# yanx27/PointASNL

Measured on AMD Instinct MI355X. Metric: point-clouds/sec fwd (Bx1024 pts, ModelNet40 cls), higher is better.
Workload: dtype f32; 1 GPU; configs[1]: ModelNet40 pointasnl_cls, 1024 pts, batch=64/GPU, seeded random weights; global_batch=64, parallelism=batch-shard x1, RCCL all-gather of logits, pipeline=prefetch, hip_graph=True, prefix_forked_at=start, prefix_levels=2, settle_replays=40, hip_hw_queues=4

## Files before the change

### include/pasnl.h

```cpp
#ifndef PASNL_H_
#define PASNL_H_

#include <stddef.h>
#include <stdint.h>

#ifdef __cplusplus
extern "C" {
#endif

#define PASNL_VERSION 100

enum {
  PASNL_OK = 0,
  PASNL_EINVAL = -1,
  PASNL_ENULL = -2,
  PASNL_EWORKSPACE = -3,
  PASNL_ELAUNCH = -4,
  PASNL_EUNSUPPORTED = -5
};

typedef void* pasnl_stream_t;

int pasnl_version(void);
const char* pasnl_strerror(int code);
// ... 102 lines not shown

int pasnl_sa_cell_packed(int b, int n, int c, int npoint, int nsample, int c1, int c2, const float* xyz, const float* feature,
                         const int* idx, const float* new_xyz, const float* w0, const float* b0, const float* w1, const float* b1,
                         const float* ww, const float* bw, const float* w0_features_packed, const float* w1_packed, float* out,
                         float* skip_max, float* new_xyz_out, float* new_feature_out, pasnl_stream_t stream);

int pasnl_max_pool_rows(int b, int n, int c, const float* x, float* out, pasnl_stream_t stream);

int pasnl_max_pool_rows_strided(int b, int n, int c, const float* x, float* out, long out_stride, pasnl_stream_t stream);

size_t pasnl_mlp3_packed_weights_bytes(int k, int n);
int pasnl_mlp3_pack_weights(int k, int n, const float* w, float* packed, pasnl_stream_t stream);
size_t pasnl_mlp3_max_pool_workspace_bytes(int b, int n, int c3);
int pasnl_mlp3_max_pool(int b, int n, int k0, int c1, int c2, int c3, const float* x, const float* w0, const float* b0,
                        const float* w1, const float* b1, const float* w2, const float* b2, float* out, long out_stride,
                        void* workspace, size_t workspace_bytes, pasnl_stream_t stream);

int pasnl_cls_tail_group_all(int b, int n, int w, int cb, int c, const float* after, const float* skip_max, const float* att,
                             const float* ws_packed, const float* bs, const float* wb_packed, const float* bb,
                             const float* wagg_packed, const float* bagg, const float* new_xyz, int c1, int c2, int c3,
                             const float* w0, const float* b0, const float* w1, const float* b1, const float* w2, const float* b2,
                             float* out, float* pooled, long pooled_stride, void* workspace, size_t workspace_bytes,
                             pasnl_stream_t stream);

size_t pasnl_bf16x3_weights_bytes(int kdim, int n);
int pasnl_bf16x3_split_weights(int kdim, int n, const float* w, void* wsplit, pasnl_stream_t stream);
int pasnl_dense_bf16x3(int rows, int kdim, int n, int lda, const float* x, const void* wsplit, const float* bias, int relu,
                       float* out, pasnl_stream_t stream);


size_t pasnl_dense_rows_workspace_bytes(int rows, int kdim, int n);
int pasnl_dense_rows(int rows, int kdim, int n, const float* x, const float* w, const float* bias, int relu, float* out,
                     void* workspace, size_t workspace_bytes, pasnl_stream_t stream);

size_t pasnl_dense_splitk_workspace_bytes(int rows, int kdim, int n);
int pasnl_dense_splitk(int rows, int kdim, int n, int lda, const float* x, const float* w, const float* bias, int relu,
                       float* out, void* workspace, size_t workspace_bytes, pasnl_stream_t stream);

int pasnl_narrow_project2(long rows0, int kdim0, int n0, const float* x0, const float* w0, const float* bias0, float* out0,
                          long rows1, int kdim1, int n1, const float* x1, const float* w1, const float* bias1, float* out1,
                          pasnl_stream_t stream);

size_t pasnl_grad_workspace_bytes(int b, int targets, long contributions);
int pasnl_gather_point_grad_det(int b, int n, int m, const float* out_g, const int* idx, float* inp_g, void* workspace,
                                size_t workspace_bytes, pasnl_stream_t stream);
int pasnl_group_point_grad_det(int b, int n, int c, int m, int nsample, const float* grad_out, const int* idx,
// ... 252 lines not shown
```

### pointasnl_amd/_hip.py

```python
import ctypes
import os

import torch

_HERE = os.path.dirname(os.path.abspath(__file__))
LIB_PATH = os.path.join(_HERE, "csrc", "libpasnl_hip.so")

SYMBOLS = [
    "pasnl_version", "pasnl_strerror", "pasnl_device_count",
    "pasnl_farthest_point_sample", "pasnl_farthest_point_sample_gather", "pasnl_gather_point", "pasnl_gather_point_grad", "pasnl_prob_sample",
    "pasnl_query_ball_point", "pasnl_sa_group", "pasnl_group_point", "pasnl_group_point_grad", "pasnl_select_top_k", "pasnl_knn_batch", "pasnl_knn_workspace_bytes", "pasnl_knn_batch_ws", "pasnl_knn_batch_ws_bg", "pasnl_knn_tree_workspace_bytes", "pasnl_knn_batch_tree", "pasnl_knn_batch_ref_workspace_bytes", "pasnl_knn_batch_ref", "pasnl_knn_distance_pick",
    "pasnl_three_nn", "pasnl_three_interpolate", "pasnl_three_interpolate_grad", "pasnl_three_weights", "pasnl_fp_interpolate_cat",
    "pasnl_nl_attention", "pasnl_nl_attention_workspace_bytes", "pasnl_nl_attention_ws", "pasnl_as_attention", "pasnl_as_reweight", "pasnl_sa_local_cell", "pasnl_sa_cell", "pasnl_sa_cell_centre0", "pasnl_sa_cell_packed", "pasnl_sa_project", "pasnl_sa_cell_pre", "pasnl_sa_cell_pre_centre0", "pasnl_sa_tail", "pasnl_sa_tail_cat", "pasnl_sa_tail_res", "pasnl_sa_tail_packed_weights_bytes", "pasnl_sa_tail_pack_weights", "pasnl_sa_tail_packed", "pasnl_decode_cell", "pasnl_decode_cell_tiled", "pasnl_decode_cell_tiled_v4", "pasnl_max_pool_rows", "pasnl_max_pool_rows_strided", "pasnl_mlp3_max_pool_workspace_bytes", "pasnl_mlp3_max_pool", "pasnl_mlp3_packed_weights_bytes", "pasnl_mlp3_pack_weights", "pasnl_dense_rows_workspace_bytes", "pasnl_dense_rows", "pasnl_dense_splitk_workspace_bytes", "pasnl_dense_splitk", "pasnl_bf16x3_weights_bytes", "pasnl_bf16x3_split_weights", "pasnl_dense_bf16x3", "pasnl_narrow_project2", "pasnl_take_neighbor0", "pasnl_as_gather", "pasnl_as_attention_qkv", "pasnl_as_attention_proj", "pasnl_as_cell_narrow", "pasnl_as_cell_wide", "pasnl_as_cell_wide_ld", "pasnl_as_reweight_x", "pasnl_grid_subsample_workspace_bytes", "pasnl_grid_subsample", "pasnl_knn_crop_workspace_bytes", "pasnl_knn_crop",
    "pasnl_scan_pick", "pasnl_knn_crop_indirect", "pasnl_crop_order_permute", "pasnl_scan_possibility_update", "pasnl_scan_scratch_init", "pasnl_scan_vote", "pasnl_scan_reproject_workspace_bytes", "pasnl_scan_reproject", "pasnl_scan_labels",
    "pasnl_scan_pick_given", "pasnl_scan_train_labels", "pasnl_scan_augment",
    "pasnl_scene_pick", "pasnl_knn_crop_scene", "pasnl_scene_pick_crop", "pasnl_scene_order_gather", "pasnl_scene_potential_update", "pasnl_scene_vote", "pasnl_scene_labels", "pasnl_confusion_matrix",
    "pasnl_window_noise", "pasnl_window_bounds", "pasnl_window_hist_bytes", "pasnl_window_count", "pasnl_window_fill", "pasnl_window_gather", "pasnl_window_vote", "pasnl_window_pool_labels",
    "pasnl_kwindow_hist_bytes", "pasnl_kwindow_count", "pasnl_kwindow_fill", "pasnl_kwindow_gather",
    "pasnl_modelnet_fps_cap", "pasnl_modelnet_fps", "pasnl_modelnet_normalize", "pasnl_modelnet_batch", "pasnl_modelnet_augment", "pasnl_modelnet_noise", "pasnl_cls_vote", "pasnl_cls_tally",
    "pasnl_cls_tail_group_all",
    "pasnl_block_key_capacity", "pasnl_block_crop_stats", "pasnl_block_grid_count", "pasnl_block_fill", "pasnl_block_gather", "pasnl_block_normalize", "pasnl_block_score_workspace_bytes", "pasnl_block_score", "pasnl_block_train_batch", "pasnl_block_train_score",
    "pasnl_kblock_crop_stats", "pasnl_kblock_grid_count", "pasnl_kblock_fill", "pasnl_kblock_gather", "pasnl_kblock_rotate",
    "pasnl_grad_workspace_bytes", "pasnl_gather_point_grad_det", "pasnl_group_point_grad_det", "pasnl_three_interpolate_grad_det",
]


class PasnlError(RuntimeError):
    pass


class PasnlUnsupported(PasnlError):
    """PASNL_EUNSUPPORTED: a valid request outside what the fused kernel covers (include/pasnl.h documents the limits).
    The cells catch it and take their op-by-op path (still HIP kernels + vendor GEMMs, never a CPU path)."""


_lib = None


def lib():
    global _lib
    if _lib is None:
        if not os.path.exists(LIB_PATH):
            raise PasnlError(
                f"{LIB_PATH} is missing: build it with `python -c 'import __graft_entry__ as g; g.build()'` "
                "(or `make -C pointasnl_amd/csrc`).  pointasnl_amd has no CPU or eager fallback.")
        _lib = ctypes.CDLL(LIB_PATH)
        _lib.pasnl_strerror.restype = ctypes.c_char_p
        _lib.pasnl_grad_workspace_bytes.restype = ctypes.c_size_t
        _lib.pasnl_knn_workspace_bytes.restype = ctypes.c_size_t
        _lib.pasnl_knn_tree_workspace_bytes.restype = ctypes.c_size_t
        _lib.pasnl_knn_batch_ref_workspace_bytes.restype = ctypes.c_size_t
        _lib.pasnl_dense_rows_workspace_bytes.restype = ctypes.c_size_t
        _lib.pasnl_bf16x3_weights_bytes.restype = ctypes.c_size_t
        _lib.pasnl_mlp3_max_pool_workspace_bytes.restype = ctypes.c_size_t
        _lib.pasnl_mlp3_packed_weights_bytes.restype = ctypes.c_size_t
        _lib.pasnl_sa_tail_packed_weights_bytes.restype = ctypes.c_size_t
        _lib.pasnl_dense_splitk_workspace_bytes.restype = ctypes.c_size_t
        _lib.pasnl_grid_subsample_workspace_bytes.restype = ctypes.c_size_t
        _lib.pasnl_knn_crop_workspace_bytes.restype = ctypes.c_size_t
        _lib.pasnl_scan_reproject_workspace_bytes.restype = ctypes.c_size_t
        _lib.pasnl_nl_attention_workspace_bytes.restype = ctypes.c_size_t
        _lib.pasnl_window_hist_bytes.restype = ctypes.c_size_t
        _lib.pasnl_kwindow_hist_bytes.restype = ctypes.c_size_t
        _lib.pasnl_block_score_workspace_bytes.restype = ctypes.c_size_t
        for s in SYMBOLS:
            getattr(_lib, s)
    return _lib


def require_device():
    if not torch.cuda.is_available():
        raise PasnlError("no HIP device visible: pointasnl_amd runs on MI355X (gfx950) only and has no CPU fallback")


def stream_ptr():
    return ctypes.c_void_p(torch.cuda.current_stream().cuda_stream)


def ptr(t, byte_offset=0):
# ... 92 lines not shown
```

### pointasnl_amd/csrc/mlp_pool.hip

```cpp
#include "common.hpp"
#include "sa_tail.hpp"

namespace pasnl {

typedef float mp_f32x16 __attribute__((ext_vector_type(16)));

__device__ __forceinline__ int mp_kappa(int t, int h) { return (t & 3) + 8 * (t >> 2) + 4 * h; }

template <int WOUT, int NB, int RB>
__device__ __forceinline__ void mp_mm(const float* xrow, int rbstride, int NBT, const float* __restrict__ Wp, const int (&loff)[NB],
                                      mp_f32x16 (&acc)[RB][NB]) {
  constexpr int BT = 8;
  float xb[2][RB][BT];
  float4 wa[2][NB][2];
  auto load = [&](int set, int bt) {
    const float* wrow = Wp + (size_t)bt * (16 * WOUT);
#pragma unroll
    for (int i = 0; i < NB; ++i) {
      wa[set][i][0] = *reinterpret_cast<const float4*>(wrow + loff[i]);
      wa[set][i][1] = *reinterpret_cast<const float4*>(wrow + loff[i] + 4);
    }
#pragma unroll
    for (int u = 0; u < BT; ++u)
#pragma unroll
// ... 40 lines not shown
  if (wave >= BLOCKS) return;
  int loff[NB];
  mp_f32x16 acc[RB][NB];
#pragma unroll
  for (int i = 0; i < NB; ++i) {
    loff[i] = (h * WOUT + (wave + NW * i) * 32 + ql) * 8;
#pragma unroll
    for (int rb = 0; rb < RB; ++rb)
#pragma unroll
      for (int r = 0; r < 16; ++r) acc[rb][i][r] = 0.f;
  }
  mp_mm<WOUT, NB, RB>(in + ql * pin + h, 32 * pin, (K + 15) >> 4, W, loff, acc);
#pragma unroll
  for (int i = 0; i < NB; ++i) {
    const int ch = (wave + NW * i) * 32 + ql;
    const float bb = bias[ch];
#pragma unroll
    for (int rb = 0; rb < RB; ++rb)
#pragma unroll
      for (int r = 0; r < 16; ++r) out[(rb * 32 + mp_kappa(r, h)) * pout + ch] = fmaxf(acc[rb][i][r] + bb, 0.f);
  }
}

template <int C1, int C2, int C3, int RB>
__device__ __forceinline__ void mlp3_tile(float* A, int pa, float* Bf, int k0, const float* __restrict__ w0, const float* __restrict__ b0,
                                          const float* __restrict__ w1, const float* __restrict__ b1, const float* __restrict__ w2,
                                          const float* __restrict__ b2, float* __restrict__ po, int wave, int ql, int h) {
  constexpr int NW = 8, PB = C1 + 1;
  mp_layer<C1, RB>(A, pa, k0, w0, b0, Bf, PB, wave, ql, h);
  __syncthreads();
  mp_layer<C2, RB>(Bf, PB, C1, w1, b1, A, pa, wave, ql, h);
  __syncthreads();
  constexpr int NB = C3 / 32 / NW;
  int loff[NB];
  mp_f32x16 acc[RB][NB];
#pragma unroll
  for (int i = 0; i < NB; ++i) {
    loff[i] = (h * C3 + (wave + NW * i) * 32 + ql) * 8;
#pragma unroll
    for (int rb = 0; rb < RB; ++rb)
#pragma unroll
      for (int r = 0; r < 16; ++r) acc[rb][i][r] = 0.f;
  }
  mp_mm<C3, NB, RB>(A + ql * pa + h, 32 * pa, C2 >> 4, w2, loff, acc);
#pragma unroll
  for (int i = 0; i < NB; ++i) {
    float mx = acc[0][i][0];
#pragma unroll
    for (int rb = 0; rb < RB; ++rb)
#pragma unroll
      for (int r = 0; r < 16; ++r) mx = fmaxf(mx, acc[rb][i][r]);
    mx = fmaxf(mx, __shfl_xor(mx, 32));
    const int ch = (wave + NW * i) * 32 + ql;
    if (h == 0) po[ch] = fmaxf(mx + b2[ch], 0.f);
  }
}

template <int C1, int C2, int C3, int RB>
__global__ __launch_bounds__(512) void mlp3_pool_kernel(int n, int k0, const float* __restrict__ x, const float* __restrict__ w0,
                                                        const float* __restrict__ b0, const float* __restrict__ w1,
                                                        const float* __restrict__ b1, const float* __restrict__ w2,
                                                        const float* __restrict__ b2, float* __restrict__ partial) {
  constexpr int NW = 8;
  static_assert(C1 % 32 == 0 && C2 % 256 == 0 && C3 % 256 == 0, "blocks of 32 channels; the two wide layers fill all eight waves");
  extern __shared__ __attribute__((aligned(16))) char smem[];
  const int pa = max((k0 + 15) & ~15, C2) | 1;
  constexpr int TR = 32 * RB;
  float* A = reinterpret_cast<float*>(smem);
  float* Bf = A + TR * pa;
  const int tid = threadIdx.x, lane = tid & 63, wave = tid >> 6, h = lane >> 5, ql = lane & 31;
  const int tile = blockIdx.x, cloud = blockIdx.y;
  {
    const int q4 = k0 >> 2;
    const float4* xc = reinterpret_cast<const float4*>(x + (size_t)cloud * n * k0);
    for (int r = wave; r < TR; r += NW) {
      const int row = min(tile * TR + r, n - 1);
      for (int q = lane; q < q4; q += 64) {
        const float4 v = xc[(size_t)row * q4 + q];
        float* d = A + r * pa + 4 * q;
        d[0] = v.x; d[1] = v.y; d[2] = v.z; d[3] = v.w;
      }
      if (lane < ((k0 + 15) & ~15) - k0) A[r * pa + k0 + lane] = 0.f;
    }
  }
  __syncthreads();
  mlp3_tile<C1, C2, C3, RB>(A, pa, Bf, k0, w0, b0, w1, b1, w2, b2, partial + ((size_t)cloud * gridDim.x + tile) * C3, wave, ql, h);
}

constexpr int TG_C = 128, TG_W = 9, TG_CB = 32, TG_K0 = TG_C + 4, TG_C2 = 256, TG_C3 = 512, TG_TR = 64;
constexpr int TG_PA = (((TG_K0 + 15) & ~15) > TG_C2 ? ((TG_K0 + 15) & ~15) : TG_C2) | 1;
constexpr int TG_TAIL_FLOATS = 2 * (TG_C + 32 + 32) * 33;
constexpr int TG_H1_FLOATS = TG_TR * (TG_C + 1);
constexpr size_t TG_LDS_BYTES = ((size_t)TG_TR * TG_PA + (TG_TAIL_FLOATS > TG_H1_FLOATS ? TG_TAIL_FLOATS : TG_H1_FLOATS)) * sizeof(float);
static_assert(TG_LDS_BYTES <= LDS_MAX_BYTES, "X rows + the tail's tiles fit one workgroup's LDS");
static_assert(TG_W <= 2 * TAIL_KS && TG_CB == 2 * TAIL_KS && TG_C % 64 == 0 && TG_C / 32 * 2 == 8, "one (channel block, row block) per wave");

__global__ __launch_bounds__(512) void tail_group_all_kernel(int n, const float* __restrict__ after, const float* __restrict__ S,
                                                             const float* __restrict__ N, const float* __restrict__ Ws,
                                                             const float* __restrict__ bs, const float* __restrict__ Wb,
                                                             const float* __restrict__ bb, const float* __restrict__ Wagg,
                                                             const float* __restrict__ bagg, const float* __restrict__ xyz3,
                                                             const float* __restrict__ w0, const float* __restrict__ b0,
                                                             const float* __restrict__ w1, const float* __restrict__ b1,
                                                             const float* __restrict__ w2, const float* __restrict__ b2,
                                                             float* __restrict__ out, float* __restrict__ partial) {
  constexpr int C = TG_C, pa = TG_PA, RPW = TG_TR / 8;
  extern __shared__ __attribute__((aligned(16))) char smem[];
  float* A = reinterpret_cast<float*>(smem);
  float* Bf = A + TG_TR * pa;
  const int tid = threadIdx.x, lane = tid & 63, wave = tid >> 6, h = lane >> 5, l32 = lane & 31;
  const int tile = blockIdx.x, cloud = blockIdx.y;
  const long cloud0 = (long)cloud * n;
  const int rb = wave >> 2;
  float* vt = Bf + rb * (C * 33);
  float* st = Bf + 2 * C * 33 + rb * (32 * 33);
  float* nt_ = Bf + 2 * (C + 32) * 33 + rb * (32 * 33);
  {
    float v[3][RPW], cx[RPW];
#pragma unroll
    for (int i = 0; i < RPW; ++i) {
      const long row = cloud0 + min(tile * TG_TR + wave * RPW + i, n - 1);
      v[0][i] = after[row * C + lane];
      v[1][i] = after[row * C + 64 + lane];
      v[2][i] = h ? N[row * TG_CB + l32] : S[row * TG_W + min(l32, TG_W - 1)];
      cx[i] = xyz3[row * 3 + max(min(lane, 3) - 1, 0)];
    }
    __builtin_amdgcn_sched_barrier(0);
    const int rr0 = (wave & 3) * RPW;
// ... 28 lines not shown
      *cell = *cell + v[i];
    }
  }
  __syncthreads();
  {
    f32x16 o;
#pragma unroll
    for (int i = 0; i < 16; ++i) o[i] = bagg[cbase + kappa(i, h)];
    o = tail_product(TailW<true>{Wagg, C, C, h, cbase + l32}, vt, l32, o);
    float* xr = A + (rb * 32 + l32) * pa + 4 + cbase;
#pragma unroll
    for (int i = 0; i < 16; ++i) xr[kappa(i, h)] = fmaxf(o[i], 0.f);
  }
  __syncthreads();
#pragma unroll
  for (int i = 0; i < RPW; ++i) {
    const int r = wave * RPW + i, row = tile * TG_TR + r;
    if (row < n) {
      float* o = out + (cloud0 + row) * C;
      o[lane] = A[r * pa + 4 + lane];
      o[64 + lane] = A[r * pa + 4 + 64 + lane];
    }
  }
  mlp3_tile<TG_C, TG_C2, TG_C3, 2>(A, pa, Bf, TG_K0, w0, b0, w1, b1, w2, b2, partial + ((size_t)cloud * gridDim.x + tile) * TG_C3, wave, l32, h);
}

__global__ __launch_bounds__(256) void mlp3_pack_kernel(int K, int N, const float* __restrict__ W, float* __restrict__ P) {
  const long total = (long)((K + 15) >> 4) * 2 * N * 2;
  for (long e = (long)blockIdx.x * 256 + threadIdx.x; e < total; e += (long)gridDim.x * 256) {
    const int half = (int)(e & 1);
    const long lane = e >> 1;
    const int n = (int)(lane % N);
    const long bh = lane / N;
    const int h = (int)(bh & 1), bt = (int)(bh >> 1);
    float v[4];
#pragma unroll
    for (int j = 0; j < 4; ++j) {
      const int k = 16 * bt + 2 * (4 * half + j) + h;
      v[j] = k < K ? W[(size_t)k * N + n] : 0.f;
    }
    reinterpret_cast<float4*>(P)[e] = make_float4(v[0], v[1], v[2], v[3]);
  }
}

template <int C1, int C2, int C3, int RB>
static int mlp3_launch(int b, int n, int k0, const float* x, const float* w0, const float* b0, const float* w1, const float* b1,
                       const float* w2, const float* b2, float* partial, hipStream_t st) {
  const int k0p = (k0 + 15) & ~15;
  const int pa = (k0p > C2 ? k0p : C2) | 1;
  const size_t lds = ((size_t)32 * RB * pa + (size_t)32 * RB * (C1 + 1)) * sizeof(float);
  if (lds > LDS_MAX_BYTES) return PASNL_EUNSUPPORTED;
  if (launch(mlp3_pool_kernel<C1, C2, C3, RB>, dim3((n + 32 * RB - 1) / (32 * RB), b), dim3(512), lds, st, n, k0, x, w0, b0, w1, b1,
             w2, b2, partial) != PASNL_OK)
    return PASNL_ELAUNCH;
  return pasnl_launch_status();
}

}

using namespace pasnl;

extern "C" size_t pasnl_mlp3_max_pool_workspace_bytes(int b, int n, int c3) {
  if (b <= 0 || n <= 0 || c3 <= 0) return 0;
  return (size_t)b * ((n + 31) / 32) * c3 * sizeof(float);
// ... 33 lines not shown
  else if (c1 == 256 && c2 == 512 && c3 == 1024) { tr = 32; rc = mlp3_launch<256, 512, 1024, 1>(b, n, k0, x, w0, b0, w1, b1, w2, b2, partial, st); }
  else return PASNL_EUNSUPPORTED;
  if (rc != PASNL_OK) return rc;
  return pasnl_max_pool_rows_strided(b, (n + tr - 1) / tr, c3, partial, out, out_stride, stream);
}

extern "C" int pasnl_cls_tail_group_all(int b, int n, int w, int cb, int c, const float* after, const float* skip_max, const float* att,
                                        const float* ws_packed, const float* bs, const float* wb_packed, const float* bb,
                                        const float* wagg_packed, const float* bagg, const float* new_xyz, int c1, int c2, int c3,
                                        const float* w0, const float* b0, const float* w1, const float* b1, const float* w2,
                                        const float* b2, float* out, float* pooled, long pooled_stride, void* workspace,
                                        size_t workspace_bytes, pasnl_stream_t stream) {
  PASNL_REQUIRE(b >= 0 && n > 0 && w > 0 && cb > 0 && c > 0 && c1 > 0 && c2 > 0 && c3 > 0 && pooled_stride >= c3, PASNL_EINVAL);
  if (b == 0) return PASNL_OK;
  PASNL_REQUIRE(after && skip_max && att && ws_packed && bs && wb_packed && bb && wagg_packed && bagg && new_xyz, PASNL_ENULL);
  PASNL_REQUIRE(w0 && b0 && w1 && b1 && w2 && b2 && out && pooled && workspace, PASNL_ENULL);
  PASNL_REQUIRE(workspace_bytes >= pasnl_mlp3_max_pool_workspace_bytes(b, n, c3), PASNL_EWORKSPACE);
  PASNL_REQUIRE(w == TG_W && cb == TG_CB && c == TG_C && c1 == TG_C && c2 == TG_C2 && c3 == TG_C3, PASNL_EUNSUPPORTED);
  PASNL_REQUIRE(b <= 65535, PASNL_EUNSUPPORTED);
  PASNL_REQUIRE((reinterpret_cast<uintptr_t>(ws_packed) | reinterpret_cast<uintptr_t>(wb_packed) | reinterpret_cast<uintptr_t>(wagg_packed) |
                 reinterpret_cast<uintptr_t>(w0) | reinterpret_cast<uintptr_t>(w1) | reinterpret_cast<uintptr_t>(w2)) % 16 == 0,
                PASNL_EUNSUPPORTED);
  const int tiles = (n + TG_TR - 1) / TG_TR;
  if (launch(tail_group_all_kernel, dim3(tiles, b), dim3(512), TG_LDS_BYTES, pasnl_hip_stream(stream), n, after, skip_max, att, ws_packed,
             bs, wb_packed, bb, wagg_packed, bagg, new_xyz, w0, b0, w1, b1, w2, b2, out, static_cast<float*>(workspace)) != PASNL_OK)
    return PASNL_ELAUNCH;
  if (pasnl_launch_status() != PASNL_OK) return PASNL_ELAUNCH;
  return pasnl_max_pool_rows_strided(b, tiles, c3, static_cast<const float*>(workspace), pooled, pooled_stride, stream);
}
```

### pointasnl_amd/models/pointasnl_cls.py

```python
import torch

from pointasnl_amd.utils import tf_util, pointasnl_util
from pointasnl_amd.utils.pointnet_util import pointnet_sa_module
from pointasnl_amd.utils.pointasnl_util import PointASNLSetAbstraction, get_repulsion_loss, sa_search, Forked


def first_layer(num_point=None):
    return dict(npoint=512, nsample=32)


def get_model(point_cloud, is_training=False, use_normal=False, bn_decay=None, weight_decay=None, num_class=40,
              adaptive_sample=False, search=None, before_head=None, fork_at="head", lazy_fork=None):
    if lazy_fork is None:
        lazy_fork = not adaptive_sample
    batch_size = point_cloud.shape[0]
    end_points = {}
    if use_normal:
        l0_xyz = point_cloud[:, :, 0:3].contiguous()
        l0_points = point_cloud[:, :, 3:6].contiguous()
    else:
        l0_xyz = point_cloud
        l0_points = point_cloud
    end_points['l0_xyz'] = l0_xyz
    as_neighbor = [12, 12] if adaptive_sample else [0, 0]

    net = torch.empty((batch_size, 1024 + 512), dtype=torch.float32, device=point_cloud.device)
    fuse3_1 = not adaptive_sample or pointasnl_util.SA_TAIL_GROUP_ALL == "always"

    search2 = []
    if isinstance(search, dict):
        search2.append(search[2])
        search = search[1]
    l1_xyz, l1_points = PointASNLSetAbstraction(l0_xyz, l0_points, npoint=512, nsample=32, mlp=[64, 64, 128],
                                                is_training=is_training, bn_decay=bn_decay, weight_decay=weight_decay,
                                                scope='layer1', as_neighbor=as_neighbor[0], search=search, xyz_concat=True,
                                                group_all=dict(mlp=[128, 256, 512], scope='layer3_1', pooled_out=net[:, 1024:]) if fuse3_1 else None,
                                                after_sampling=None if search2 else lambda xyz1: search2.append(
                                                    Forked(lambda: sa_search(xyz1, None, 128, 64), lazy=lazy_fork)))
    end_points['l1_xyz'] = l1_xyz
    l2_xyz, l2_points = PointASNLSetAbstraction(l1_xyz, l1_points, npoint=128, nsample=64, mlp=[128, 128, 256],
                                                is_training=is_training, bn_decay=bn_decay, weight_decay=weight_decay,
                                                scope='layer2', as_neighbor=as_neighbor[1], search=search2[0], xyz_concat=True,
                                                after_cell=before_head if fork_at == "cell2" else None,
                                                before_after_conv=before_head if fork_at == "conv2" else None)
    end_points['l2_xyz'] = l1_xyz
    if before_head is not None and fork_at == "head":
        before_head()
    if getattr(l1_points, "group_all_pooled", None) is None:
        _, l3_points_res, _ = pointnet_sa_module(l1_xyz, l1_points, npoint=None, radius=None, nsample=None,
                                                 mlp=[128, 256, 512], mlp2=None, group_all=True, is_training=is_training,
                                                 bn_decay=bn_decay, scope='layer3_1', pooled_out=net[:, 1024:])
    _, l3_points, _ = pointnet_sa_module(l2_xyz, l2_points, npoint=None, radius=None, nsample=None,
                                         mlp=[256, 512, 1024], mlp2=None, group_all=True, is_training=is_training,
                                         bn_decay=bn_decay, scope='layer3_2', pooled_out=net[:, :1024])

    net = tf_util.fully_connected(net, 512, bn=True, is_training=is_training, scope='fc1', bn_decay=bn_decay)
    net = tf_util.dropout(net, keep_prob=0.4, is_training=is_training, scope='dp1')
    net = tf_util.fully_connected(net, 256, bn=True, is_training=is_training, scope='fc2', bn_decay=bn_decay)
    net = tf_util.dropout(net, keep_prob=0.4, is_training=is_training, scope='dp2')
# ... 17 lines not shown
```

### pointasnl_amd/utils/pointasnl_util.py

```python

import ctypes

import torch

from pointasnl_amd import _hip
from pointasnl_amd import tf_sampling, tf_grouping, nearest_neighbors
from pointasnl_amd.tf_interpolate import three_nn, three_interpolate, three_weights, fp_interpolate_cat
from pointasnl_amd.utils import tf_util, pointnet_util

NL_KEY_PARTS = True
NL_VARIANT = 0


KNN_TIE_ORDER = "reference"


def knn_query(k, support_pts, query_pts, out=None, max_workgroups=None):
    return nearest_neighbors.knn_batch(support_pts, query_pts, k, omp=True, dtype=torch.int32, tie_order=KNN_TIE_ORDER, out=out,
                                       max_workgroups=max_workgroups)


def _gather_rows(points, idx):
    return tf_grouping.group_point(points, idx.unsqueeze(-1)).squeeze(2)

# ... 17 lines not shown
    grouped_xyz = tf_grouping.group_point(src_xyz, point_indices)
    grouped_feature = tf_grouping.group_point(feature, point_indices)
    if use_xyz:
        grouped_feature = torch.cat([grouped_xyz, grouped_feature], dim=-1)
    return grouped_xyz, grouped_feature, point_indices


def sa_group(xyz, feature, idx, new_xyz):
    b, n, c = feature.shape
    _, p, k = idx.shape
    xyz, feature, idx, new_xyz = xyz.contiguous(), feature.contiguous(), idx.contiguous(), new_xyz.contiguous()
    new_point = torch.empty((b, p, k, 6 + c), dtype=torch.float32, device=xyz.device)
    skip = torch.empty((b, p, 6 + c), dtype=torch.float32, device=xyz.device)
    _hip.launch("pasnl_sa_group", "sa_group", b, n, c, p, k, _hip.ptr(xyz), _hip.ptr(feature), _hip.ptr(idx),
                _hip.ptr(new_xyz), _hip.ptr(new_point), _hip.ptr(skip))
    return new_point, skip


SELF_KNN_RATIO = 2
SA_TAIL_MIN_ROWS = 2048
FP_HEAD_FUSED = True
SA_CELL_PACKED = True
SA_TAIL_PACKED = True
SA_TAIL_GROUP_ALL = True
SA_TAIL_FUSED = True
SA_CELL_GATHER = True
SA_CELL_SINGLE = True
SA_CELL_WIDE = True
LOCAL_CELL_FUSED = True


def _local_cell_supported(w, mlp, nsample):
    if not LOCAL_CELL_FUSED or nsample % 32:
        return False
    wide = (256, 512) if SA_CELL_WIDE else ()
    if len(mlp) == 3:
        return mlp[0] == mlp[1] and mlp[0] in (16, 32, 64, 128) + wide
    return len(mlp) == 2 and mlp[0] in (32, 64, 128) + wide


def sa_local_cell(new_point, mlp, is_training, bn_decay, weight_decay, bn):
    b, p, k, w = new_point.shape
    c1, c2 = mlp[0], mlp[1]
    st = tf_util.store()
    with tf_util.variable_scope('conv0'):
        w0, b0 = st.layer(w, c1, bn, weight_decay)
    with tf_util.variable_scope('conv1'):
# ... 85 lines not shown
    _hip.launch("pasnl_sa_cell", "sa_cell", b, n, c, p, k, ck, ck, _hip.ptr(xyz), _hip.ptr(feature), _hip.ptr(idx),
                _hip.ptr(new_xyz), _hip.ptr(w0), _hip.ptr(b0), _hip.ptr(w1), _hip.ptr(b1), _hip.ptr(ww), _hip.ptr(bw),
                _hip.ptr(out), _hip.ptr(skip))
    return view, skip


SA_CELL_PREPROJECT = True
SA_PREPROJECT_REUSE = 8


def sa_cell_pre_supported(b, n, c, npoint, nsample, mlp, feature):
    if not (SA_CELL_PREPROJECT and len(mlp) == 3 and mlp[0] == mlp[1] and mlp[0] in (32, 64, 128)):
        return False
    if c % 4 or c > 128 or nsample % 32 or npoint * nsample < SA_PREPROJECT_REUSE * n:
        return False
    if feature.is_contiguous() and feature.data_ptr() % 16:
        return False
    return not (mlp[0] == 128 and nsample == 32 and b * npoint <= 2048)


def sa_cell_pre(xyz, feature, idx, new_xyz, mlp, is_training, bn_decay, weight_decay, bn):
    b, n, c = feature.shape
    _, p, k = idx.shape
    xyz, feature, idx = xyz.contiguous(), feature.contiguous(), idx.contiguous()
    w0, b0, w1, b1, ww, bw, ck = _sa_cell_weights(6 + c, mlp, bn, weight_decay)
    proj = torch.empty((b, n, ck), dtype=torch.float32, device=xyz.device)
    _hip.launch("pasnl_sa_project", "sa_project", b, n, c, ck, _hip.ptr(xyz), _hip.ptr(feature), _hip.ptr(w0), _hip.ptr(b0),
                _hip.ptr(proj))
    out = torch.empty((b, p, ck, 32), dtype=torch.float32, device=xyz.device)
    skip = torch.empty((b, p, 6 + c), dtype=torch.float32, device=xyz.device)
    if new_xyz is None:
        cen = torch.empty((b, p, 3), dtype=torch.float32, device=xyz.device)
        nf = torch.empty((b, p, 3 + c), dtype=torch.float32, device=xyz.device)
        _hip.launch("pasnl_sa_cell_pre_centre0", "sa_cell_pre", b, n, c, p, k, ck, ck, _hip.ptr(xyz), _hip.ptr(feature),
                    _hip.ptr(proj), _hip.ptr(idx), _hip.ptr(w0), _hip.ptr(w1), _hip.ptr(b1), _hip.ptr(ww), _hip.ptr(bw),
                    _hip.ptr(out), _hip.ptr(skip), _hip.ptr(cen), _hip.ptr(nf))
        return out, skip, cen, nf
    new_xyz = new_xyz.contiguous()
    _hip.launch("pasnl_sa_cell_pre", "sa_cell_pre", b, n, c, p, k, ck, ck, _hip.ptr(xyz), _hip.ptr(feature), _hip.ptr(proj),
                _hip.ptr(idx), _hip.ptr(new_xyz), _hip.ptr(w0), _hip.ptr(w1), _hip.ptr(b1), _hip.ptr(ww), _hip.ptr(bw),
                _hip.ptr(out), _hip.ptr(skip))
    return out, skip


def weight_net_hidden(xyz, hidden_units, scope, is_training, bn_decay=None, weight_decay=None, activation_fn="relu"):
    with tf_util.variable_scope(scope):
        net = xyz
        for i, num_hidden_units in enumerate(hidden_units):
            net = tf_util.conv2d(net, num_hidden_units, [1, 1], padding='VALID', stride=[1, 1], bn=True,
                                 is_training=is_training, activation_fn=activation_fn, scope='wconv%d' % (i),
                                 bn_decay=bn_decay, weight_decay=weight_decay)
# ... 354 lines not shown
    fp = Forked(lambda: tf_sampling.farthest_point_sample_gather(npoint, xyz), slot=slot)

    def join():
        fps_idx, new_xyz = fp.get()
        k_all = _resolved(knn_all)
        idx = _gather_index_rows(k_all, fps_idx)
        if k_all.shape[2] != nsample:
            idx = idx[:, :, :nsample].contiguous()
        return new_xyz, None, idx
    return Deferred(join)


def _tail_packed(st, w):
    key = "@tailpk:%x" % w.data_ptr()
    if key not in st._folded:
        wc = w.contiguous()
        pk = torch.empty(int(_hip.lib().pasnl_sa_tail_packed_weights_bytes(wc.shape[0], wc.shape[1])) // 4, dtype=torch.float32,
                         device=w.device)
        _hip.launch("pasnl_sa_tail_pack_weights", "sa_tail_pack", int(wc.shape[0]), int(wc.shape[1]), _hip.ptr(wc), _hip.ptr(pk))
        st._folded[key] = (pk, w)
    return st._folded[key][0]


def PointASNLSetAbstraction(xyz, feature, npoint, nsample, mlp, is_training, bn_decay, weight_decay, scope, bn=True,
                            use_knn=True, radius=None, as_neighbor=8, NL=True, search=None, after_sampling=None,
                            xyz_concat=False, after_cell=None, before_after_conv=None, residual=None, group_all=None):
    ga_weights = None
    if (group_all is not None and SA_TAIL_GROUP_ALL and SA_TAIL_FUSED and SA_TAIL_PACKED and NL and residual is None and not is_training
            and mlp[-1] == 128 and tuple(group_all['mlp']) == (128, 256, 512)):
        with tf_util.variable_scope(group_all['scope']):
            ga_weights = pointnet_util.group_all_weights(group_all['mlp'], 3 + mlp[-1], 1, bn)
    with tf_util.variable_scope(scope):
        batch_size, num_points, num_channel = feature.shape
        new_xyz, _, idx = _resolved(search) if search is not None else sa_search(xyz, feature, npoint, nsample, use_knn, radius)
        new_feature = feature
        nl_channel = mlp[-1]

        fused = _local_cell_supported(6 + num_channel, mlp, nsample)
        centre0 = False
        if num_points != npoint and as_neighbor == 0:
            xyz, feature, idx = xyz.contiguous(), feature.contiguous(), idx.contiguous()

            def take0():
                nx = torch.empty((batch_size, npoint, 3), dtype=torch.float32, device=xyz.device)
                nf = torch.empty((batch_size, npoint, 3 + num_channel), dtype=torch.float32, device=xyz.device)
                _hip.launch("pasnl_take_neighbor0", "take_neighbor0", batch_size, num_points, num_channel, npoint, nsample,
                            _hip.ptr(xyz), _hip.ptr(feature), _hip.ptr(idx), _hip.ptr(nx), _hip.ptr(nf))
                return nx, nf
            centre0 = (CENTRE0 and fused and SA_CELL_GATHER and npoint <= num_points
                       and (num_channel <= 128 or (SA_CELL_WIDE and mlp[0] in (256, 512) and nsample == 32)))
            if not centre0:
                new_xyz, new_feature = take0()
        elif num_points != npoint and AS_FUSED and as_neighbor <= 16:
            tf_util._require_inference(is_training)
# ... 64 lines not shown
            w_in = skip_spatial.shape[-1]
            with tf_util.variable_scope('skip'):
                ws, bs = st.layer(w_in, c_out, bn, weight_decay)
            if NL:
                with tf_util.variable_scope(scope), tf_util.variable_scope('conv_back_project'):
                    wb, bb = st.layer(cb, c_out, bn, weight_decay)
            with tf_util.variable_scope('aggregation'):
                wagg, bagg = st.layer(c_out, c_out, bn, weight_decay)
            rows = batch_size * npoint
            after, skip_spatial = after.contiguous(), skip_spatial.contiguous()
            att = att.contiguous() if NL else None
            out = torch.empty((batch_size, npoint, c_out), dtype=torch.float32, device=xyz.device)
            args = (rows, int(w_in), int(cb if NL else 0), int(c_out), _hip.ptr(after), _hip.ptr(skip_spatial),
                    _hip.ptr(att), _hip.ptr(ws), _hip.ptr(bs), _hip.ptr(wb if NL else None),
                    _hip.ptr(bb if NL else None), _hip.ptr(wagg), _hip.ptr(bagg), _hip.ptr(out))
            try:
                if SA_TAIL_PACKED:
                    pk = [_tail_packed(st, m) if m is not None else None for m in (ws, wb if NL else None, wagg)]
                    cat = None
                    if ga_weights is not None and (int(w_in), int(cb)) == (9, 32) and new_xyz.shape[1] == npoint:
                        new_xyz = new_xyz.contiguous()
                        gmlp = group_all['mlp']
                        pooled = pointnet_util.group_all_pooled(group_all.get('pooled_out'), batch_size, gmlp[-1], xyz.device)
                        wsb = pointnet_util.group_all_workspace(batch_size, npoint, gmlp[-1], xyz.device)
                        _hip.launch("pasnl_cls_tail_group_all", "sa_tail_group_all", batch_size, npoint, int(w_in), int(cb), int(c_out),
                                    *args[4:7], _hip.ptr(pk[0]), args[8], _hip.ptr(pk[1]), args[10], _hip.ptr(pk[2]), args[12],
                                    _hip.ptr(new_xyz), gmlp[0], gmlp[1], gmlp[2], *[_hip.ptr(t) for t in ga_weights], args[13],
                                    _hip.ptr(pooled), ctypes.c_long(pooled.stride(0) if batch_size > 1 else gmlp[-1]),
                                    _hip.ptr(wsb), ctypes.c_size_t(wsb.numel()))
                        out.group_all_pooled = pooled
                        return new_xyz, out
                    if xyz_concat and XYZ_CONCAT:
                        new_xyz = new_xyz.contiguous()
                        cat = torch.empty((batch_size, npoint, 4 + c_out), dtype=torch.float32, device=xyz.device)
                    res_c = residual.contiguous() if residual is not None else None
                    _hip.launch("pasnl_sa_tail_packed", "sa_tail", *args[:7], _hip.ptr(pk[0]), args[8], _hip.ptr(pk[1]), args[10],
                                _hip.ptr(pk[2]), args[12], _hip.ptr(res_c), _hip.ptr(new_xyz if cat is not None else None),
                                _hip.ptr(cat), args[13])
                    residual = None
                    if cat is not None:
                        out.xyz_concat = (new_xyz, cat)
                elif residual is not None:
                    residual = residual.contiguous()
                    _hip.launch("pasnl_sa_tail_res", "sa_tail", *args[:-1], _hip.ptr(residual), args[-1])
                    residual = None
                elif xyz_concat and XYZ_CONCAT:
# ... 135 lines not shown
```

Measured before the change: 57070 point-clouds/s.

## Fold next layer's conv0 projection and final max-pool into group-all tail kernel

The fused layer1 tail plus group-all kernel now also computes layer2's first-conv projection table from the rows it already holds in LDS, using MFMA with a packed weight layout. The next SA cell reuses that table instead of launching its own sa_project kernel. The separate max-pool reduction launch is replaced by a last-block-done pattern: per-cloud atomic counters pick the last tile block, which reduces the partial maxima in-kernel. This removes two kernel launches and one re-read of the layer1 features, at the cost of extra per-block work, atomics with relaxed loads, and a persistent counter workspace that must stay zeroed.

```diff
diff --git a/include/pasnl.h b/include/pasnl.h
--- a/include/pasnl.h
+++ b/include/pasnl.h
@@ -148,6 +148,16 @@
                              const float* w0, const float* b0, const float* w1, const float* b1, const float* w2, const float* b2,
                              float* out, float* pooled, long pooled_stride, void* workspace, size_t workspace_bytes,
                              pasnl_stream_t stream);
+
+size_t pasnl_cls_tail_group_all_fold_workspace_bytes(int b, int n, int c3);
+size_t pasnl_cls_project_packed_weights_bytes(int c, int c1);
+int pasnl_cls_project_pack_weights(int c, int c1, const float* w0, const float* b0, float* packed, pasnl_stream_t stream);
+int pasnl_cls_tail_group_all_fold(int b, int n, int w, int cb, int c, const float* after, const float* skip_max, const float* att,
+                                  const float* ws_packed, const float* bs, const float* wb_packed, const float* bb,
+                                  const float* wagg_packed, const float* bagg, const float* new_xyz, int c1, int c2, int c3,
+                                  const float* w0, const float* b0, const float* w1, const float* b1, const float* w2,
+                                  const float* b2, int cp, const float* proj_w_packed, float* out, float* pooled, long pooled_stride,
+                                  float* proj, void* workspace, size_t workspace_bytes, pasnl_stream_t stream);
 
 size_t pasnl_bf16x3_weights_bytes(int kdim, int n);
 int pasnl_bf16x3_split_weights(int kdim, int n, const float* w, void* wsplit, pasnl_stream_t stream);
diff --git a/pointasnl_amd/_hip.py b/pointasnl_amd/_hip.py
--- a/pointasnl_amd/_hip.py
+++ b/pointasnl_amd/_hip.py
@@ -18,7 +18,8 @@
     "pasnl_window_noise", "pasnl_window_bounds", "pasnl_window_hist_bytes", "pasnl_window_count", "pasnl_window_fill", "pasnl_window_gather", "pasnl_window_vote", "pasnl_window_pool_labels",
     "pasnl_kwindow_hist_bytes", "pasnl_kwindow_count", "pasnl_kwindow_fill", "pasnl_kwindow_gather",
     "pasnl_modelnet_fps_cap", "pasnl_modelnet_fps", "pasnl_modelnet_normalize", "pasnl_modelnet_batch", "pasnl_modelnet_augment", "pasnl_modelnet_noise", "pasnl_cls_vote", "pasnl_cls_tally",
-    "pasnl_cls_tail_group_all",
+    "pasnl_cls_tail_group_all", "pasnl_cls_tail_group_all_fold", "pasnl_cls_tail_group_all_fold_workspace_bytes",
+    "pasnl_cls_project_pack_weights", "pasnl_cls_project_packed_weights_bytes",
     "pasnl_block_key_capacity", "pasnl_block_crop_stats", "pasnl_block_grid_count", "pasnl_block_fill", "pasnl_block_gather", "pasnl_block_normalize", "pasnl_block_score_workspace_bytes", "pasnl_block_score", "pasnl_block_train_batch", "pasnl_block_train_score",
     "pasnl_kblock_crop_stats", "pasnl_kblock_grid_count", "pasnl_kblock_fill", "pasnl_kblock_gather", "pasnl_kblock_rotate",
     "pasnl_grad_workspace_bytes", "pasnl_gather_point_grad_det", "pasnl_group_point_grad_det", "pasnl_three_interpolate_grad_det",
@@ -55,6 +56,8 @@
         _lib.pasnl_mlp3_max_pool_workspace_bytes.restype = ctypes.c_size_t
         _lib.pasnl_mlp3_packed_weights_bytes.restype = ctypes.c_size_t
         _lib.pasnl_sa_tail_packed_weights_bytes.restype = ctypes.c_size_t
+        _lib.pasnl_cls_tail_group_all_fold_workspace_bytes.restype = ctypes.c_size_t
+        _lib.pasnl_cls_project_packed_weights_bytes.restype = ctypes.c_size_t
         _lib.pasnl_dense_splitk_workspace_bytes.restype = ctypes.c_size_t
         _lib.pasnl_grid_subsample_workspace_bytes.restype = ctypes.c_size_t
         _lib.pasnl_knn_crop_workspace_bytes.restype = ctypes.c_size_t
diff --git a/pointasnl_amd/csrc/mlp_pool.hip b/pointasnl_amd/csrc/mlp_pool.hip
--- a/pointasnl_amd/csrc/mlp_pool.hip
+++ b/pointasnl_amd/csrc/mlp_pool.hip
@@ -86,7 +86,7 @@
   }
 }
 
-template <int C1, int C2, int C3, int RB>
+template <int C1, int C2, int C3, int RB, bool WRITE_THROUGH = false>
 __device__ __forceinline__ void mlp3_tile(float* A, int pa, float* Bf, int k0, const float* __restrict__ w0, const float* __restrict__ b0,
                                           const float* __restrict__ w1, const float* __restrict__ b1, const float* __restrict__ w2,
                                           const float* __restrict__ b2, float* __restrict__ po, int wave, int ql, int h) {
@@ -116,7 +116,11 @@
       for (int r = 0; r < 16; ++r) mx = fmaxf(mx, acc[rb][i][r]);
     mx = fmaxf(mx, __shfl_xor(mx, 32));
     const int ch = (wave + NW * i) * 32 + ql;
-    if (h == 0) po[ch] = fmaxf(mx + b2[ch], 0.f);
+    if (h == 0) {
+      const float v = fmaxf(mx + b2[ch], 0.f);
+      if constexpr (WRITE_THROUGH) __hip_atomic_store(po + ch, v, __ATOMIC_RELAXED, __HIP_MEMORY_SCOPE_AGENT);
+      else po[ch] = v;
+    }
   }
 }
 
@@ -157,8 +161,49 @@
 constexpr int TG_H1_FLOATS = TG_TR * (TG_C + 1);
 constexpr size_t TG_LDS_BYTES = ((size_t)TG_TR * TG_PA + (TG_TAIL_FLOATS > TG_H1_FLOATS ? TG_TAIL_FLOATS : TG_H1_FLOATS)) * sizeof(float);
 static_assert(TG_LDS_BYTES <= LDS_MAX_BYTES, "X rows + the tail's tiles fit one workgroup's LDS");
+constexpr int TG_PROJ_CHUNKS = (8 + TG_C + 31) / 32;
 static_assert(TG_W <= 2 * TAIL_KS && TG_CB == 2 * TAIL_KS && TG_C % 64 == 0 && TG_C / 32 * 2 == 8, "one (channel block, row block) per wave");
 
+__device__ __forceinline__ void tg_project(const float* xr, const float* __restrict__ wp, float* __restrict__ prow, int rows_left,
+                                           int blk, int l32, int h) {
+  const float* wl = wp + ((size_t)h * TG_C + blk * 32 + l32) * 8;
+  const float* xh = xr + 16 * h - 4;
+  mp_f32x16 acc;
+#pragma unroll
+  for (int r = 0; r < 16; ++r) acc[r] = 0.f;
+  float4 wall[TG_PROJ_CHUNKS][4];
+#pragma unroll
+  for (int ch = 0; ch < TG_PROJ_CHUNKS; ++ch)
+#pragma unroll
+    for (int q = 0; q < 4; ++q) wall[ch][q] = *reinterpret_cast<const float4*>(wl + (size_t)(2 * ch + (q >> 1)) * (16 * TG_C) + 4 * (q & 1));
+  __builtin_amdgcn_sched_barrier(0);
+#pragma unroll
+  for (int ch = 0; ch < TG_PROJ_CHUNKS; ++ch) {
+    const float4 (&w)[4] = wall[ch];
+#pragma unroll
+    for (int t = 0; t < 16; ++t) {
+      float x;
+      if (ch == 0 && t < 8) {
+        const float v = *(h ? xh + t : xr + (t >= 3 && t <= 5 ? t - 2 : 0));
+        x = (t == 6 && !h) ? 1.f : v;
+      } else if (ch == TG_PROJ_CHUNKS - 1) {
+        x = *((t < 8 && !h) ? xh + 32 * ch + t : xr);
+      } else {
+        x = xh[32 * ch + t];
+      }
+      const float4 q = w[t >> 2];
+      const float wv = (t & 3) == 0 ? q.x : ((t & 3) == 1 ? q.y : ((t & 3) == 2 ? q.z : q.w));
+      acc = __builtin_amdgcn_mfma_f32_32x32x2f32(x, wv, acc, 0, 0, 0);
+    }
+  }
+#pragma unroll
+  for (int r = 0; r < 16; ++r) {
+    const int row = mp_kappa(r, h);
+    if (row < rows_left) prow[(size_t)row * TG_C + blk * 32 + l32] = acc[r];
+  }
+}
+
+template <bool FOLD>
 __global__ __launch_bounds__(512) void tail_group_all_kernel(int n, const float* __restrict__ after, const float* __restrict__ S,
                                                              const float* __restrict__ N, const float* __restrict__ Ws,
                                                              const float* __restrict__ bs, const float* __restrict__ Wb,
@@ -167,7 +212,9 @@
                                                              const float* __restrict__ w0, const float* __restrict__ b0,
                                                              const float* __restrict__ w1, const float* __restrict__ b1,
                                                              const float* __restrict__ w2, const float* __restrict__ b2,
-                                                             float* __restrict__ out, float* __restrict__ partial) {
+                                                             float* __restrict__ out, float* partial, const float* __restrict__ wproj,
+                                                             float* __restrict__ proj, float* __restrict__ pooled, long pooled_stride,
+                                                             unsigned* counters) {
   constexpr int C = TG_C, pa = TG_PA, RPW = TG_TR / 8;
   extern __shared__ __attribute__((aligned(16))) char smem[];
   float* A = reinterpret_cast<float*>(smem);
@@ -242,7 +289,24 @@
       o[64 + lane] = A[r * pa + 4 + 64 + lane];
     }
   }
-  mlp3_tile<TG_C, TG_C2, TG_C3, 2>(A, pa, Bf, TG_K0, w0, b0, w1, b1, w2, b2, partial + ((size_t)cloud * gridDim.x + tile) * TG_C3, wave, l32, h);
+  if constexpr (FOLD) tg_project(A + (rb * 32 + l32) * pa, wproj, proj + (cloud0 + tile * TG_TR + rb * 32) * C, n - tile * TG_TR - rb * 32, wave & 3, l32, h);
+  mlp3_tile<TG_C, TG_C2, TG_C3, 2, FOLD>(A, pa, Bf, TG_K0, w0, b0, w1, b1, w2, b2, partial + ((size_t)cloud * gridDim.x + tile) * TG_C3, wave, l32, h);
+  if constexpr (FOLD) {
+    int* last = reinterpret_cast<int*>(Bf);
+    asm volatile("s_waitcnt vmcnt(0)" ::: "memory");
+    __syncthreads();
+    if (tid == 0) {
+      const unsigned seen = atomicAdd(&counters[cloud], 1u);
+      *last = seen == gridDim.x - 1;
+      if (*last) counters[cloud] = 0;
+    }
+    __syncthreads();
+    if (!*last) return;
+    float* pc = partial + (size_t)cloud * gridDim.x * TG_C3 + tid;
+    float m = __hip_atomic_load(pc, __ATOMIC_RELAXED, __HIP_MEMORY_SCOPE_AGENT);
+    for (unsigned t = 1; t < gridDim.x; ++t) m = fmaxf(m, __hip_atomic_load(pc + (size_t)t * TG_C3, __ATOMIC_RELAXED, __HIP_MEMORY_SCOPE_AGENT));
+    pooled[(size_t)cloud * pooled_stride + tid] = m;
+  }
 }
 
 __global__ __launch_bounds__(256) void mlp3_pack_kernel(int K, int N, const float* __restrict__ W, float* __restrict__ P) {
@@ -260,6 +324,24 @@
       v[j] = k < K ? W[(size_t)k * N + n] : 0.f;
     }
     reinterpret_cast<float4*>(P)[e] = make_float4(v[0], v[1], v[2], v[3]);
+  }
+}
+
+__global__ __launch_bounds__(256) void sa_project_pack_kernel(int c, int c1, const float* __restrict__ w0, const float* __restrict__ b0,
+                                                              float* __restrict__ P) {
+  const long total = (long)((8 + c + 31) & ~31) * c1;
+  for (long e = (long)blockIdx.x * 256 + threadIdx.x; e < total; e += (long)gridDim.x * 256) {
+    const int u = (int)(e & 7);
+    const long lane = e >> 3;
+    const int col = (int)(lane % c1);
+    const long bh = lane / c1;
+    const int h = (int)(bh & 1), s = (int)(bh >> 1) * 8 + u;
+    const int i = 32 * (s >> 4) + 16 * h + (s & 15);
+    float v = 0.f;
+    if (i >= 3 && i < 6) v = w0[(size_t)i * c1 + col];
+    else if (i == 6) v = b0[col];
+    else if (i >= 8 && i < 8 + c) v = w0[(size_t)(i - 2) * c1 + col];
+    P[e] = v;
   }
 }
 
@@ -339,9 +421,63 @@
                  reinterpret_cast<uintptr_t>(w0) | reinterpret_cast<uintptr_t>(w1) | reinterpret_cast<uintptr_t>(w2)) % 16 == 0,
                 PASNL_EUNSUPPORTED);
   const int tiles = (n + TG_TR - 1) / TG_TR;
-  if (launch(tail_group_all_kernel, dim3(tiles, b), dim3(512), TG_LDS_BYTES, pasnl_hip_stream(stream), n, after, skip_max, att, ws_packed,
-             bs, wb_packed, bb, wagg_packed, bagg, new_xyz, w0, b0, w1, b1, w2, b2, out, static_cast<float*>(workspace)) != PASNL_OK)
+  if (launch(tail_group_all_kernel<false>, dim3(tiles, b), dim3(512), TG_LDS_BYTES, pasnl_hip_stream(stream), n, after, skip_max, att,
+             ws_packed, bs, wb_packed, bb, wagg_packed, bagg, new_xyz, w0, b0, w1, b1, w2, b2, out, static_cast<float*>(workspace),
+             static_cast<const float*>(nullptr), static_cast<float*>(nullptr), static_cast<float*>(nullptr), 0L,
+             static_cast<unsigned*>(nullptr)) != PASNL_OK)
     return PASNL_ELAUNCH;
   if (pasnl_launch_status() != PASNL_OK) return PASNL_ELAUNCH;
   return pasnl_max_pool_rows_strided(b, tiles, c3, static_cast<const float*>(workspace), pooled, pooled_stride, stream);
 }
+
+static size_t tg_counter_bytes(int b) { return ((size_t)b * sizeof(unsigned) + 255) & ~(size_t)255; }
+
+extern "C" size_t pasnl_cls_tail_group_all_fold_workspace_bytes(int b, int n, int c3) {
+  if (b <= 0 || n <= 0 || c3 <= 0) return 0;
+  return tg_counter_bytes(b) + (size_t)b * ((n + TG_TR - 1) / TG_TR) * c3 * sizeof(float);
+}
+
+extern "C" size_t pasnl_cls_project_packed_weights_bytes(int c, int c1) {
+  if (c <= 0 || c1 <= 0) return 0;
+  return (size_t)((8 + c + 31) & ~31) * c1 * sizeof(float);
+}
+
+extern "C" int pasnl_cls_project_pack_weights(int c, int c1, const float* w0, const float* b0, float* packed, pasnl_stream_t stream) {
+  PASNL_REQUIRE(c > 0 && c1 > 0, PASNL_EINVAL);
+  PASNL_REQUIRE(w0 && b0 && packed, PASNL_ENULL);
+  PASNL_REQUIRE(reinterpret_cast<uintptr_t>(packed) % 16 == 0, PASNL_EUNSUPPORTED);
+  const long total = (long)((8 + c + 31) & ~31) * c1;
+  const long g = (total + 255) / 256;
+  hipLaunchKernelGGL(sa_project_pack_kernel, dim3((unsigned)(g > 4096 ? 4096 : g)), dim3(256), 0, pasnl_hip_stream(stream), c, c1, w0, b0,
+                     packed);
+  return pasnl_launch_status();
+}
+
+extern "C" int pasnl_cls_tail_group_all_fold(int b, int n, int w, int cb, int c, const float* after, const float* skip_max,
+                                             const float* att, const float* ws_packed, const float* bs, const float* wb_packed,
+                                             const float* bb, const float* wagg_packed, const float* bagg, const float* new_xyz, int c1,
+                                             int c2, int c3, const float* w0, const float* b0, const float* w1, const float* b1,
+                                             const float* w2, const float* b2, int cp, const float* proj_w_packed, float* out,
+                                             float* pooled, long pooled_stride, float* proj, void* workspace, size_t workspace_bytes,
+                                             pasnl_stream_t stream) {
+  PASNL_REQUIRE(b >= 0 && n > 0 && w > 0 && cb > 0 && c > 0 && c1 > 0 && c2 > 0 && c3 > 0 && cp > 0 && pooled_stride >= c3, PASNL_EINVAL);
+  if (b == 0) return PASNL_OK;
+  PASNL_REQUIRE(after && skip_max && att && ws_packed && bs && wb_packed && bb && wagg_packed && bagg && new_xyz, PASNL_ENULL);
+  PASNL_REQUIRE(w0 && b0 && w1 && b1 && w2 && b2 && proj_w_packed && out && pooled && proj && workspace, PASNL_ENULL);
+  PASNL_REQUIRE(workspace_bytes >= pasnl_cls_tail_group_all_fold_workspace_bytes(b, n, c3), PASNL_EWORKSPACE);
+  PASNL_REQUIRE(w == TG_W && cb == TG_CB && c == TG_C && c1 == TG_C && c2 == TG_C2 && c3 == TG_C3 && cp == TG_C, PASNL_EUNSUPPORTED);
+  PASNL_REQUIRE(b <= 65535, PASNL_EUNSUPPORTED);
+  PASNL_REQUIRE((reinterpret_cast<uintptr_t>(ws_packed) | reinterpret_cast<uintptr_t>(wb_packed) | reinterpret_cast<uintptr_t>(wagg_packed) |
+                 reinterpret_cast<uintptr_t>(w0) | reinterpret_cast<uintptr_t>(w1) | reinterpret_cast<uintptr_t>(w2) |
+                 reinterpret_cast<uintptr_t>(proj_w_packed)) % 16 == 0,
+                PASNL_EUNSUPPORTED);
+  PASNL_REQUIRE(reinterpret_cast<uintptr_t>(workspace) % 4 == 0, PASNL_EUNSUPPORTED);
+  const int tiles = (n + TG_TR - 1) / TG_TR;
+  unsigned* counters = static_cast<unsigned*>(workspace);
+  float* partial = reinterpret_cast<float*>(static_cast<char*>(workspace) + tg_counter_bytes(b));
+  if (launch(tail_group_all_kernel<true>, dim3(tiles, b), dim3(512), TG_LDS_BYTES, pasnl_hip_stream(stream), n, after, skip_max, att,
+             ws_packed, bs, wb_packed, bb, wagg_packed, bagg, new_xyz, w0, b0, w1, b1, w2, b2, out, partial, proj_w_packed, proj, pooled,
+             pooled_stride, counters) != PASNL_OK)
+    return PASNL_ELAUNCH;
+  return pasnl_launch_status();
+}
diff --git a/pointasnl_amd/models/pointasnl_cls.py b/pointasnl_amd/models/pointasnl_cls.py
--- a/pointasnl_amd/models/pointasnl_cls.py
+++ b/pointasnl_amd/models/pointasnl_cls.py
@@ -35,6 +35,7 @@
                                                 is_training=is_training, bn_decay=bn_decay, weight_decay=weight_decay,
                                                 scope='layer1', as_neighbor=as_neighbor[0], search=search, xyz_concat=True,
                                                 group_all=dict(mlp=[128, 256, 512], scope='layer3_1', pooled_out=net[:, 1024:]) if fuse3_1 else None,
+                                                next_conv0=dict(mlp=[128, 128, 256], scope='layer2') if fuse3_1 else None,
                                                 after_sampling=None if search2 else lambda xyz1: search2.append(
                                                     Forked(lambda: sa_search(xyz1, None, 128, 64), lazy=lazy_fork)))
     end_points['l1_xyz'] = l1_xyz
diff --git a/pointasnl_amd/utils/pointasnl_util.py b/pointasnl_amd/utils/pointasnl_util.py
--- a/pointasnl_amd/utils/pointasnl_util.py
+++ b/pointasnl_amd/utils/pointasnl_util.py
@@ -63,7 +63,7 @@
 FP_HEAD_FUSED = True
 SA_CELL_PACKED = True
 SA_TAIL_PACKED = True
-SA_TAIL_GROUP_ALL = True
+SA_TAIL_GROUP_ALL = "fold"
 SA_TAIL_FUSED = True
 SA_CELL_GATHER = True
 SA_CELL_SINGLE = True
@@ -195,11 +195,17 @@
 def sa_cell_pre(xyz, feature, idx, new_xyz, mlp, is_training, bn_decay, weight_decay, bn):
     b, n, c = feature.shape
     _, p, k = idx.shape
+    table = getattr(feature, "conv0_table", None)
+    if table is not None and table[2] is not xyz:
+        table = None
     xyz, feature, idx = xyz.contiguous(), feature.contiguous(), idx.contiguous()
     w0, b0, w1, b1, ww, bw, ck = _sa_cell_weights(6 + c, mlp, bn, weight_decay)
-    proj = torch.empty((b, n, ck), dtype=torch.float32, device=xyz.device)
-    _hip.launch("pasnl_sa_project", "sa_project", b, n, c, ck, _hip.ptr(xyz), _hip.ptr(feature), _hip.ptr(w0), _hip.ptr(b0),
-                _hip.ptr(proj))
+    if table is not None and table[0] is w0 and table[1] is b0 and tuple(table[3].shape) == (b, n, ck):
+        proj = table[3]
+    else:
+        proj = torch.empty((b, n, ck), dtype=torch.float32, device=xyz.device)
+        _hip.launch("pasnl_sa_project", "sa_project", b, n, c, ck, _hip.ptr(xyz), _hip.ptr(feature), _hip.ptr(w0), _hip.ptr(b0),
+                    _hip.ptr(proj))
     out = torch.empty((b, p, ck, 32), dtype=torch.float32, device=xyz.device)
     skip = torch.empty((b, p, 6 + c), dtype=torch.float32, device=xyz.device)
     if new_xyz is None:
@@ -600,14 +606,41 @@
     return st._folded[key][0]
 
 
+def _project_packed(st, w0, b0):
+    key = "@projpk:%x:%x" % (w0.data_ptr(), b0.data_ptr())
+    if key not in st._folded:
+        c, c1 = int(w0.shape[0]) - 6, int(w0.shape[1])
+        pk = torch.empty(int(_hip.lib().pasnl_cls_project_packed_weights_bytes(c, c1)) // 4, dtype=torch.float32, device=w0.device)
+        _hip.launch("pasnl_cls_project_pack_weights", "project_pack", c, c1, _hip.ptr(w0), _hip.ptr(b0), _hip.ptr(pk))
+        st._folded[key] = (pk, w0, b0)
+    return st._folded[key][0]
+
+
+_TAIL_FOLD_WS = {}
+
+
+def _tail_fold_workspace(b, n, c3, device):
+    nbytes = int(_hip.lib().pasnl_cls_tail_group_all_fold_workspace_bytes(b, n, c3))
+    key = (device.index, torch.cuda.current_stream().cuda_stream)
+    bufs = _TAIL_FOLD_WS.setdefault(key, [])
+    if not bufs or bufs[-1].numel() < nbytes:
+        bufs.append(torch.zeros(max(nbytes, 256), dtype=torch.uint8, device=device))
+    return bufs[-1]
+
+
 def PointASNLSetAbstraction(xyz, feature, npoint, nsample, mlp, is_training, bn_decay, weight_decay, scope, bn=True,
                             use_knn=True, radius=None, as_neighbor=8, NL=True, search=None, after_sampling=None,
-                            xyz_concat=False, after_cell=None, before_after_conv=None, residual=None, group_all=None):
-    ga_weights = None
+                            xyz_concat=False, after_cell=None, before_after_conv=None, residual=None, group_all=None,
+                            next_conv0=None):
+    ga_weights, next_w = None, None
     if (group_all is not None and SA_TAIL_GROUP_ALL and SA_TAIL_FUSED and SA_TAIL_PACKED and NL and residual is None and not is_training
             and mlp[-1] == 128 and tuple(group_all['mlp']) == (128, 256, 512)):
         with tf_util.variable_scope(group_all['scope']):
             ga_weights = pointnet_util.group_all_weights(group_all['mlp'], 3 + mlp[-1], 1, bn)
+        nmlp = next_conv0['mlp'] if next_conv0 is not None else ()
+        if SA_TAIL_GROUP_ALL == "fold" and SA_CELL_PREPROJECT and len(nmlp) == 3 and nmlp[0] == nmlp[1] == 128:
+            with tf_util.variable_scope(next_conv0['scope']):
+                next_w = _sa_cell_weights(6 + mlp[-1], nmlp, bn, weight_decay)[:2]
     with tf_util.variable_scope(scope):
         batch_size, num_points, num_channel = feature.shape
         new_xyz, _, idx = _resolved(search) if search is not None else sa_search(xyz, feature, npoint, nsample, use_knn, radius)
@@ -718,6 +751,19 @@
                         new_xyz = new_xyz.contiguous()
                         gmlp = group_all['mlp']
                         pooled = pointnet_util.group_all_pooled(group_all.get('pooled_out'), batch_size, gmlp[-1], xyz.device)
+                        if next_w is not None:
+                            cp = int(next_w[0].shape[1])
+                            proj = torch.empty((batch_size, npoint, cp), dtype=torch.float32, device=xyz.device)
+                            wsb = _tail_fold_workspace(batch_size, npoint, gmlp[-1], xyz.device)
+                            _hip.launch("pasnl_cls_tail_group_all_fold", "sa_tail_group_all", batch_size, npoint, int(w_in), int(cb),
+                                        int(c_out), *args[4:7], _hip.ptr(pk[0]), args[8], _hip.ptr(pk[1]), args[10], _hip.ptr(pk[2]),
+                                        args[12], _hip.ptr(new_xyz), gmlp[0], gmlp[1], gmlp[2], *[_hip.ptr(t) for t in ga_weights], cp,
+                                        _hip.ptr(_project_packed(st, *next_w)), args[13], _hip.ptr(pooled),
+                                        ctypes.c_long(pooled.stride(0) if batch_size > 1 else gmlp[-1]), _hip.ptr(proj), _hip.ptr(wsb),
+                                        ctypes.c_size_t(wsb.numel()))
+                            out.group_all_pooled = pooled
+                            out.conv0_table = (next_w[0], next_w[1], new_xyz, proj)
+                            return new_xyz, out
                         wsb = pointnet_util.group_all_workspace(batch_size, npoint, gmlp[-1], xyz.device)
                         _hip.launch("pasnl_cls_tail_group_all", "sa_tail_group_all", batch_size, npoint, int(w_in), int(cb), int(c_out),
                                     *args[4:7], _hip.ptr(pk[0]), args[8], _hip.ptr(pk[1]), args[10], _hip.ptr(pk[2]), args[12],
```

New measurement: 57340 point-clouds/s, median of 6. About the same (+0.5%).
